# sabarim/STEm-Seg

Hardware: AMD Instinct MI355X
Metric: clips/sec (T=8, 480p) embed+cluster (higher is better)
Workload: dtype f16x3: fp32 emulated from 2 fp16 terms per operand (22-bit operand significands; fp32 has 24), power-of-two operand scaling, 3 fp16 MFMA products per fp32 product, fp32 accumulate; |activation| >= 2.6e5 -> non-finite, flagged on the device, clip re-run in bf16x6

## Files before the change

stem-seg_amd/csrc/conv_igemm.hip:

```cpp
#include "common.h"
#include <algorithm>
#include <cstdlib>
#include <type_traits>

#define STEMSEG_F16X3_ACT_SCALE 0.25f

#ifndef SS_F16_WPLANES
#define SS_F16_WPLANES 2
#endif
#ifndef SS_EXPERIMENTS
#if defined(SS_PROBE) || defined(SS_X6_WMODE_SMALLG) || defined(SS_X6_SPREAD) || defined(SS_X6_SPREAD_DIV)
#error "SS_PROBE / SS_X6_WMODE_SMALLG / SS_X6_SPREAD / SS_X6_SPREAD_DIV are experiment switches: add -DSS_EXPERIMENTS"
#endif
#define SS_X6_WMODE_SMALLG -1
#define SS_X6_SPREAD 1
#define SS_X6_SPREAD_DIV 1
#define SS_PROBE 0
#else
#ifndef SS_X6_WMODE_SMALLG
#define SS_X6_WMODE_SMALLG -1
#endif
#ifndef SS_X6_SPREAD
#define SS_X6_SPREAD 1
#endif
#ifndef SS_X6_SPREAD_DIV
#define SS_X6_SPREAD_DIV 1
#endif

#ifndef SS_PROBE
#define SS_PROBE 0
#endif

#endif

#if SS_PROBE == 5
#define SS_CHUNK_SYNC() do { } while (0)
#else
#define SS_CHUNK_SYNC() __syncthreads()
#endif

namespace stemseg {

typedef float f32x16 __attribute__((ext_vector_type(16)));

#ifndef STEMSEG_MIN_WG4
#define STEMSEG_MIN_WG4 4
#endif
constexpr int MIN_WG4 = STEMSEG_MIN_WG4;

struct ConvKParams {
    const float* in;
    int64_t in_cs, in_ts, in_ys, in_limit;
    int in_H;
    const float* wpk;
    const float* bias;
    float* out;
    int64_t out_cs, out_ts, out_ys;
    int Cin, Cout, T, H, W;
    int tiles_x, tiles_y;
    int vec4;
    int chunks_per_split;
    int64_t out_split_stride;
    int relu;
    const float* res;
    int64_t res_cs, res_ts, res_ys;
    int dec_H, dec_W;
    int vec_epi;
    int t_fastest;
    int flat_t;
    int T_all;
    int n_co;
    double* gn_part;
    int gn_cpg, gn_cap, gn_slot0;
    int* gn_used_host;
    int nb;
    int64_t in_bs, out_bs, gn_bs;
    unsigned int* out_p16;
};

template <int KT_, int KH_, int KW_, int CK_, int MI_, int NI_, int WM_, int WN_, int COLS_, bool PIPE_ = false, int BF_ = 0, bool DB_ = false,
          int PMAX_ = 0, bool GL_ = false, int BLK_ = 0>
struct ConvCfg {
    static constexpr bool PIPE = PIPE_, BF = BF_ != 0, X6 = BF_ >= 2, F16 = BF_ == 3, DB = DB_, FLAT = PMAX_ > 0, GL = GL_;
    static_assert(BF_ == 0 || BF_ == 2 || BF_ == 3, "precision: 0 fp32-input MFMA, 2 bf16x6, 3 f16x3");
    static constexpr int NPL = BF_ == 2 ? 3 : (BF_ == 3 ? SS_F16_WPLANES : 2);
    static constexpr int NPA = 3;
    static constexpr int NPX = BF_ == 2 ? 3 : 2;
    static constexpr int NPROD = BF_ == 2 ? 6 : 3;
    static constexpr int PMAX = PMAX_;
    static constexpr int KT = KT_, KH = KH_, KW = KW_, CK = CK_, MI = MI_, NI = NI_, WM = WM_, WN = WN_, COLS = COLS_;
    static constexpr int TAPS = KT * KH * KW;
    static constexpr int NTHREADS = 64 * WM * WN;
    static constexpr int MT = WM * MI * 32;
    static constexpr int NSEG = WN * NI;
    static constexpr bool BLK = BLK_ > 0;
    static constexpr int NLIVE = BLK ? BLK_ * COLS_ : NSEG;
    static constexpr int ROWS = BLK ? 4 * BLK_ : NSEG / COLS;
    static constexpr int TW = BLK ? 8 * COLS_ : COLS_ * 32;
    static constexpr int RH = ROWS + KH - 1;
    static constexpr int XL = (TW + KW - 1 + 3) / 4;
    static constexpr int XP = BLK ? ((4 * XL + 23) / 32) * 32 + 8 : 4 * XL;
    static constexpr int NT = NSEG * 32;
    static constexpr int FL = NT + 2 * PMAX + 8;
    static constexpr int IN_CH_STRIDE = FLAT ? KT * FL : KT * RH * XP;
    static constexpr int IN_PAIR_STRIDE = PMAX_ > 0 ? KT * (WN_ * NI_ * 32 + 2 * PMAX_ + 8) : KT * RH * XP;
    static constexpr int IN_PLANE_STRIDE = (CK / 2) * IN_PAIR_STRIDE;
    static constexpr int IN_FLOATS = X6 ? NPX * IN_PLANE_STRIDE : CK * IN_CH_STRIDE;
    static constexpr int TPG = TAPS >= 27 ? 4 : ((TAPS >= 9 && CK_ < 16) ? 2 : 1);
    static constexpr int CPH = 8 / TPG;
    static constexpr int NTG = (TAPS + TPG - 1) / TPG;
    static constexpr int NCG = BF ? CK / (2 * CPH) : 1;
    static constexpr int G = NTG * NCG;
    static constexpr int W_FLOATS = BF ? NPL * G * 2 * MT * 4 : CK * TAPS * MT;
    static constexpr int GA = (G + 1) / 2;
    static constexpr int WMODE = (BF_ >= 2 && G <= 2) ? (SS_X6_WMODE_SMALLG >= 0 ? SS_X6_WMODE_SMALLG : (BF_ == 3 ? 1 : ((WM * WN >= 8 || MI * NI < 8) ? 2 : 0))) : 0;
    static constexpr bool SP = WMODE == 1, LA = WMODE == 2;
    static constexpr int IN_ALL = IN_FLOATS;
    static constexpr int BUF_FLOATS = IN_ALL + W_FLOATS;
    static constexpr int LDS_FLOATS = BUF_FLOATS * (DB ? 2 : 1);
    static_assert(!BF || CK % (2 * CPH) == 0, "split-staged: a chunk holds whole k-groups");
    static_assert(BLK || NSEG % COLS == 0, "segments must fill whole rows");
    static_assert(!BLK || (BF_ >= 2 && PMAX_ == 0 && NI_ == 2 && NLIVE <= NSEG && NLIVE > NSEG - NI_ && XP % 32 == 8 && XP >= 4 * XL), "block tiles: split-staged, the last wave may lack its second block");
    static_assert(CK % 4 == 0 || (DB && GL_ && CK == 2 && !BF), "channel chunk is a multiple of the packed sub-chunk (4), or one channel pair (GL)");
    static_assert(LDS_FLOATS * 4 <= (X6 ? 160 : 80) * 1024, "two workgroups per CU (x6 eight-wave tiles: one)");
    static_assert(!X6 || (!DB && !GL && G >= 2 && CK % 2 == 0), "x6: 2-D / 3-D tiles, two weight phases");
    static_assert(!FLAT || (KH == 3 && KW == 3 && PMAX % 4 == 0), "flat tiles: 3x3 taps");
    static_assert(DB == GL_, "two LDS buffers are the direct-to-LDS form");
    static_assert(!GL || (DB && !BF), "direct-to-LDS staging is the double-buffered fp32 form");
    static constexpr int NWAVES = WM * WN;
    static constexpr int MIN_WG = X6 ? (MI * NI > 8 ? 1 : NWAVES >= 8 ? 2 : (LDS_FLOATS * 4 * 2 <= 160 * 1024 ? NWAVES / 2 : NWAVES / 4))
                                     : ((GL && LDS_FLOATS * 4 * 4 <= 140 * 1024 && MI * NI <= 4) ? MIN_WG4 : ((GL && LDS_FLOATS * 4 * 3 <= 160 * 1024) ? 3 : 2));
};

__device__ __forceinline__ void split_pair_f16(const float x0, const float x1, unsigned int& hw, unsigned int& lw) {
    const float qs = STEMSEG_F16X3_ACT_SCALE, ks = 2048.0f;
    unsigned int h, l;
    float r0, r1;
    asm("v_fma_mixlo_f16 %0, %1, %2, 0" : "=v"(h) : "v"(x0), "s"(qs));
    asm("v_fma_mixhi_f16 %0, %1, %2, 0" : "+v"(h) : "v"(x1), "s"(qs));
    asm("v_fma_mix_f32 %0, %1, %2, -%3 op_sel_hi:[0,0,1]" : "=v"(r0) : "v"(x0), "s"(qs), "v"(h));
    asm("v_fma_mix_f32 %0, %1, %2, -%3 op_sel:[0,0,1] op_sel_hi:[0,0,1]" : "=v"(r1) : "v"(x1), "s"(qs), "v"(h));
    asm("v_fma_mixlo_f16 %0, %1, %2, 0" : "=v"(l) : "v"(r0), "s"(ks));
    asm("v_fma_mixhi_f16 %0, %1, %2, 0" : "+v"(l) : "v"(r1), "s"(ks));
    hw = h;
    lw = l;
}

template <class C>
__global__ __launch_bounds__(C::NTHREADS, C::MIN_WG) void conv_igemm_kernel(const ConvKParams p) {
    __shared__ __attribute__((aligned(16))) float smem[C::LDS_FLOATS];
    float* const in_lds = smem;
    float* const w_lds = smem + C::IN_ALL;

    const int tid = threadIdx.x;
    const int lane = tid & 63;
    const int wave = __builtin_amdgcn_readfirstlane(tid >> 6);
    const int wm = wave / C::WN, wn = wave % C::WN;
    const int half = lane >> 5, l31 = lane & 31;

    int bx;
    {
        const int nwg = gridDim.x, xcd = blockIdx.x & 7, q = nwg >> 3, r = nwg & 7;
        bx = (xcd < r ? xcd * (q + 1) : r * (q + 1) + (xcd - r) * q) + (blockIdx.x >> 3);
    }
    const int co_tile = bx % p.n_co;
    bx /= p.n_co;
    int tx, ty, t;
    if (C::KT > 1 && p.t_fastest) {
        t = bx % p.T;
        bx /= p.T;
        tx = bx % p.tiles_x;
        ty = bx / p.tiles_x;
    } else {
        tx = bx % p.tiles_x;
        bx /= p.tiles_x;
        ty = bx % p.tiles_y;
        t = bx / p.tiles_y;
    }
    const int x0 = C::FLAT ? 0 : tx * C::TW, y0 = C::FLAT ? 0 : ty * C::ROWS;
    auto seg_row = [](const int sN, const int l) __attribute__((always_inline)) { return C::BLK ? (sN / C::COLS) * 4 + (l >> 3) : sN / C::COLS; };
    auto seg_col = [](const int sN, const int l) __attribute__((always_inline)) { return C::BLK ? (sN % C::COLS) * 8 + (l & 7) : (sN % C::COLS) * 32 + l; };
    const bool ni1_live = !C::BLK || (wn * C::NI + 1 < C::NLIVE);
    const int pitch = (int)p.in_ys;
    const int F0 = pitch + tx * C::NT;
    const int co0 = co_tile * C::MT;

    f32x16 acc[C::MI][C::NI];
#pragma unroll
    for (int mi = 0; mi < C::MI; ++mi)
#pragma unroll
        for (int ni = 0; ni < C::NI; ++ni)
#pragma unroll
            for (int r = 0; r < 16; ++r) acc[mi][ni][r] = 0.f;

    const float* a_ptr = w_lds + half * C::MT + wm * (C::MI * 32) + l31;
    const float* b_ptr[C::NI];
#pragma unroll
    for (int ni = 0; ni < C::NI; ++ni) {
        const int s = wn * C::NI + ni;
        b_ptr[ni] = C::FLAT ? in_lds + half * C::IN_CH_STRIDE + s * 32 + l31 + 3
                            : in_lds + half * C::IN_CH_STRIDE + seg_row(s, l31) * C::XP + seg_col(s, l31);
    }

    const unsigned int* b_ptr6[C::NI];
#pragma unroll
    for (int ni = 0; ni < C::NI; ++ni) {
        const int s = wn * C::NI + ni;
        b_ptr6[ni] = C::FLAT ? reinterpret_cast<const unsigned int*>(in_lds) + half * (C::CPH / 2) * C::IN_PAIR_STRIDE + s * 32 + l31 + 3
                             : reinterpret_cast<const unsigned int*>(in_lds) + half * (C::CPH / 2) * C::IN_PAIR_STRIDE + seg_row(min(s, C::NLIVE - 1), l31) * C::XP + seg_col(min(s, C::NLIVE - 1), l31);
    }
    const float* in_tile = p.in + (int64_t)blockIdx.y * p.in_bs + (int64_t)t * p.in_ts + x0;
    const int64_t tile_base = (int64_t)t * p.in_ts + x0;

    constexpr int XQ = C::XP / 4;
    constexpr int NQ = C::FLAT ? C::IN_FLOATS / 4 : C::CK * C::KT * C::RH * XQ;
    constexpr int MQ = C::MT / 4;
    constexpr int NWQ = C::BF ? C::NPL * C::G * 2 * C::MT : C::CK * C::TAPS * MQ;
    constexpr int IN_PT = (NQ + C::NTHREADS - 1) / C::NTHREADS, W_PT = (NWQ + C::NTHREADS - 1) / C::NTHREADS;
    auto fetch_in = [&](int c0, int q) -> float4 {
        if constexpr (C::FLAT) {
            constexpr int FQ = C::FL / 4;
            const int j4 = q % FQ, rr = q / FQ, dt = rr % C::KT, c = rr / C::KT;
            const int f = F0 - pitch - 4 + 4 * j4;
            const int64_t rel = (int64_t)(c0 + c) * p.in_cs + (int64_t)dt * p.in_ts + f;
            float4 v = make_float4(0.f, 0.f, 0.f, 0.f);
            if (c0 + c < p.Cin && f >= 0 && 4 * j4 < C::NT + 2 * pitch + 8 && tile_base + rel + 4 <= p.in_limit)
                v = *reinterpret_cast<const float4*>(in_tile + rel);
            return v;
        }
        const int xq = q % XQ;
        int rr = q / XQ;
        const int r = rr % C::RH;
        rr /= C::RH;
        const int dt = rr % C::KT;
        const int c = rr / C::KT;
        const int yy = min(y0 + r, p.in_H - 1);
        const int64_t rel = (int64_t)(c0 + c) * p.in_cs + (int64_t)dt * p.in_ts + (int64_t)yy * p.in_ys + xq * 4;
        float4 v = make_float4(0.f, 0.f, 0.f, 0.f);
        if (c0 + c < p.Cin && tile_base + rel + 4 <= p.in_limit) v = *reinterpret_cast<const float4*>(in_tile + rel);
        return v;
    };
    auto fetch_w = [&](int c0, int q) -> float4 {
        const int mq = q % MQ;
        if constexpr (C::CK == 2) {
            const int row2 = q / MQ, tap = row2 >> 1, e = row2 & 1;
            const float* wsrc2 = p.wpk + ((int64_t)(c0 / 4) * (C::TAPS * 4) + tap * 4 + ((c0 >> 1) & 1) * 2 + e) * p.Cout + co0;
            float4 v2 = make_float4(0.f, 0.f, 0.f, 0.f);
            if (c0 + e < p.Cin && co0 + mq * 4 < p.Cout) v2 = *reinterpret_cast<const float4*>(wsrc2 + mq * 4);
            return v2;
        }
        const int row = q / MQ;
        const int ch = c0 + (row / (C::TAPS * 4)) * 4 + (row & 3);
        const float* wsrc = p.wpk + (int64_t)(c0 / 4) * (C::TAPS * 4) * p.Cout + co0;
        float4 v = make_float4(0.f, 0.f, 0.f, 0.f);
        if (ch < p.Cin && co0 + mq * 4 < p.Cout) v = *reinterpret_cast<const float4*>(wsrc + (int64_t)row * p.Cout + mq * 4);
        return v;
    };
    auto addr_in = [&](int c0, int q) -> const float* {
        int64_t rel;
        if constexpr (C::FLAT) {
            constexpr int FQ = C::FL / 4;
            const int j4 = q % FQ, rr = q / FQ, dt = rr % C::KT, c = rr / C::KT;
            const int f = max(F0 - pitch - 4 + 4 * j4, 0);
            rel = (int64_t)(c0 + c) * p.in_cs + (int64_t)dt * p.in_ts + f;
        } else {
            const int xq = q % XQ;
            int rr = q / XQ;
            const int r = rr % C::RH;
            rr /= C::RH;
            const int dt = rr % C::KT;
            const int c = rr / C::KT;
            const int yy = min(y0 + r, p.in_H - 1);
            rel = (int64_t)(c0 + c) * p.in_cs + (int64_t)dt * p.in_ts + (int64_t)yy * p.in_ys + xq * 4;
        }
        const int64_t last = p.in_limit - 4 - tile_base;
        return in_tile + (rel < last ? rel : last);
    };
    auto addr_w = [&](int c0, int q) -> const float* {
        const int mq = q % MQ;
        if constexpr (C::CK == 2) {
            const int row2 = q / MQ, tap = row2 >> 1, e = row2 & 1;
            return p.wpk + ((int64_t)(c0 / 4) * (C::TAPS * 4) + tap * 4 + ((c0 >> 1) & 1) * 2 + e) * p.Cout + co0 + mq * 4;
        } else {
            const int row = q / MQ;
            return p.wpk + (int64_t)(c0 / 4) * (C::TAPS * 4) * p.Cout + co0 + (int64_t)row * p.Cout + mq * 4;
        }
    };
    auto glds_chunk = [&](int c0, const int off) {
        typedef const __attribute__((address_space(1))) void* gptr_t;
        typedef __attribute__((address_space(3))) void* lptr_t;
#pragma unroll
        for (int k = 0; k < IN_PT; ++k) {
            const int q = tid + k * C::NTHREADS;
            if (q < NQ) __builtin_amdgcn_global_load_lds((gptr_t)addr_in(c0, q), (lptr_t)(in_lds + off + (q - lane) * 4), 16, 0, 0);
        }
#pragma unroll
        for (int k = 0; k < W_PT; ++k) {
            const int q = tid + k * C::NTHREADS;
            if (q < NWQ) __builtin_amdgcn_global_load_lds((gptr_t)addr_w(c0, q), (lptr_t)(w_lds + off + (q - lane) * 4), 16, 0, 0);
        }
    };
    auto stage_direct = [&](int c0) {
        if (p.vec4) {
            for (int q = tid; q < NQ; q += C::NTHREADS) *reinterpret_cast<float4*>(in_lds + q * 4) = fetch_in(c0, q);
        } else if constexpr (!C::FLAT) {
            constexpr int NE = C::CK * C::KT * C::RH * C::XP;
            for (int q = tid; q < NE; q += C::NTHREADS) {
                const int xx = q % C::XP;
                int rr = q / C::XP;
                const int r = rr % C::RH;
                rr /= C::RH;
                const int dt = rr % C::KT;
                const int c = rr / C::KT;
                const int yy = min(y0 + r, p.in_H - 1);
                const int64_t rel = (int64_t)(c0 + c) * p.in_cs + (int64_t)dt * p.in_ts + (int64_t)yy * p.in_ys + xx;
                float v = 0.f;
                if (c0 + c < p.Cin && tile_base + rel < p.in_limit) v = in_tile[rel];
                in_lds[q] = v;
            }
        }
        for (int q = tid; q < NWQ; q += C::NTHREADS) *reinterpret_cast<float4*>(w_lds + q * 4) = fetch_w(c0, q);
    };

    auto split3 = [](const float x, unsigned int& h, unsigned int& m, unsigned int& l) {
        if constexpr (C::F16) {
            const float xs = x * STEMSEG_F16X3_ACT_SCALE;
            const _Float16 fh = (_Float16)xs;
            const _Float16 fl = (_Float16)((xs - (float)fh) * 2048.0f);
            h = *reinterpret_cast<const unsigned short*>(&fh);
            m = *reinterpret_cast<const unsigned short*>(&fl);
            l = 0;
        } else {
            const __bf16 bh = (__bf16)x;
            const float r1 = x - (float)bh;
            const __bf16 bm = (__bf16)r1;
            const __bf16 bl = (__bf16)(r1 - (float)bm);
            h = *reinterpret_cast<const unsigned short*>(&bh);
            m = *reinterpret_cast<const unsigned short*>(&bm);
            l = *reinterpret_cast<const unsigned short*>(&bl);
        }
    };
    constexpr int FQ6 = C::FL / 4;
    constexpr int XL6 = C::XL;
    constexpr int NQ6 = C::FLAT ? (C::CK / 2) * C::KT * FQ6 : (C::CK / 2) * C::KT * C::RH * XL6;
    auto in6_lds = [](const int q) __attribute__((always_inline)) { return C::BLK ? (q / XL6) * C::XP + (q % XL6) * 4 : q * 4; };
    constexpr int IN_PT6 = C::X6 ? (NQ6 + C::NTHREADS - 1) / C::NTHREADS : 1;
    constexpr int NWQ_A = C::NPL * C::GA * 2 * C::MT, NWQ6 = C::NPL * C::G * 2 * C::MT;
    auto in6_rel = [&](int q, int& c) -> int64_t {
        if constexpr (C::FLAT) {
            const int j4 = q % FQ6, rr = q / FQ6, dt = rr % C::KT;
            c = 2 * (rr / C::KT);
            const int f = F0 - pitch - 4 + 4 * j4;
            if (f < 0 || 4 * j4 >= C::NT + 2 * pitch + 8) return -1;
            return (int64_t)c * p.in_cs + (int64_t)dt * p.in_ts + f;
        }
        const int xq = q % XL6;
        int rr = q / XL6;
        const int r = rr % C::RH;
        rr /= C::RH;
        const int dt = rr % C::KT;
        c = 2 * (rr / C::KT);
        const int yy = min(y0 + r, p.in_H - 1);
        return (int64_t)c * p.in_cs + (int64_t)dt * p.in_ts + (int64_t)yy * p.in_ys + xq * 4;
    };
    auto fetch_in6 = [&](int c0, int q, float4& v0, float4& v1) {
        int c;
        const int64_t rel0 = in6_rel(q, c);
        const int64_t rel = rel0 + (int64_t)c0 * p.in_cs;
        v0 = v1 = make_float4(0.f, 0.f, 0.f, 0.f);
        if (rel0 < 0) return;
        if (c0 + c < p.Cin && tile_base + rel + 4 <= p.in_limit) v0 = *reinterpret_cast<const float4*>(in_tile + rel);
        if (c0 + c + 1 < p.Cin && tile_base + rel + p.in_cs + 4 <= p.in_limit) v1 = *reinterpret_cast<const float4*>(in_tile + rel + p.in_cs);
    };
    unsigned int in6_voff[IN_PT6];
    int in6_clim[IN_PT6];
    const int64_t in6_room = (p.in_limit - 4 - tile_base) * 4;
    if constexpr (C::X6) {
#pragma unroll
        for (int k = 0; k < IN_PT6; ++k) {
            const int q = tid + k * C::NTHREADS;
            int c = 0;
            const int64_t rel0 = q < NQ6 ? in6_rel(q, c) : 0;
            const int64_t rel = rel0 < 0 ? 0 : rel0;
            in6_voff[k] = (unsigned int)(rel * 4);
            const int64_t slack = in6_room - rel * 4;
            const int64_t by_room = slack < 0 ? 0 : slack / (p.in_cs * 4) + 1;
            in6_clim[k] = (q < NQ6 && rel0 >= 0) ? (int)min((int64_t)(p.Cin - c), by_room) : 0;
        }
    }
    typedef float f32x4 __attribute__((ext_vector_type(4)));
    auto fetch_in6_fast = [&](int c0, int k, f32x4& v0, f32x4& v1) __attribute__((always_inline)) {
#if SS_PROBE == 1
        return;
#endif
        const char* base = reinterpret_cast<const char*>(in_tile) + (int64_t)c0 * p.in_cs * 4;
        const unsigned int cs4 = (unsigned int)(p.in_cs * 4);
        v0 = *reinterpret_cast<const f32x4*>(base + (c0 < in6_clim[k] ? in6_voff[k] : 0u));
        v1 = *reinterpret_cast<const f32x4*>(base + (c0 + 1 < in6_clim[k] ? in6_voff[k] + cs4 : 0u));
    };
    auto store_in6 = [&](int q, const float4& v0, const float4& v1) {
        unsigned int h0, m0, l0, h1, m1, l1;
        uint4 ph, pm, pl;
        if constexpr (C::F16) {
            split_pair_f16(v0.x, v1.x, ph.x, pm.x); split_pair_f16(v0.y, v1.y, ph.y, pm.y);
            split_pair_f16(v0.z, v1.z, ph.z, pm.z); split_pair_f16(v0.w, v1.w, ph.w, pm.w);
            unsigned int* d16 = reinterpret_cast<unsigned int*>(in_lds) + in6_lds(q);
            *reinterpret_cast<uint4*>(d16) = ph;
            *reinterpret_cast<uint4*>(d16 + C::IN_PLANE_STRIDE) = pm;
            return;
        }
        split3(v0.x, h0, m0, l0); split3(v1.x, h1, m1, l1); ph.x = h0 | (h1 << 16); pm.x = m0 | (m1 << 16); pl.x = l0 | (l1 << 16);
        split3(v0.y, h0, m0, l0); split3(v1.y, h1, m1, l1); ph.y = h0 | (h1 << 16); pm.y = m0 | (m1 << 16); pl.y = l0 | (l1 << 16);
        split3(v0.z, h0, m0, l0); split3(v1.z, h1, m1, l1); ph.z = h0 | (h1 << 16); pm.z = m0 | (m1 << 16); pl.z = l0 | (l1 << 16);
        split3(v0.w, h0, m0, l0); split3(v1.w, h1, m1, l1); ph.w = h0 | (h1 << 16); pm.w = m0 | (m1 << 16); pl.w = l0 | (l1 << 16);
        unsigned int* d = reinterpret_cast<unsigned int*>(in_lds) + in6_lds(q);
        *reinterpret_cast<uint4*>(d) = ph;
        *reinterpret_cast<uint4*>(d + C::IN_PLANE_STRIDE) = pm;
        if constexpr (C::NPX == 3) *reinterpret_cast<uint4*>(d + 2 * C::IN_PLANE_STRIDE) = pl;
    };
    auto store_in6_masked = [&](int c0, int k, const f32x4& r0, const f32x4& r1) __attribute__((always_inline)) {
        const bool ok0 = c0 < in6_clim[k], ok1 = c0 + 1 < in6_clim[k];
        float4 v0, v1;
        v0.x = ok0 ? r0.x : 0.f; v0.y = ok0 ? r0.y : 0.f; v0.z = ok0 ? r0.z : 0.f; v0.w = ok0 ? r0.w : 0.f;
        v1.x = ok1 ? r1.x : 0.f; v1.y = ok1 ? r1.y : 0.f; v1.z = ok1 ? r1.z : 0.f; v1.w = ok1 ? r1.w : 0.f;
        store_in6(tid + k * C::NTHREADS, v0, v1);
    };
    auto stage_in6_direct = [&](int c0) {
        if (p.vec4) {
            for (int q = tid; q < NQ6; q += C::NTHREADS) {
                float4 v0, v1;
                fetch_in6(c0, q, v0, v1);
                store_in6(q, v0, v1);
            }
        } else if constexpr (!C::FLAT) {
            constexpr int NE6 = (C::CK / 2) * C::KT * C::RH * C::XP;
            for (int q = tid; q < NE6; q += C::NTHREADS) {
                const int xx = q % C::XP;
                int rr = q / C::XP;
                const int r = rr % C::RH;
                rr /= C::RH;
                const int dt = rr % C::KT;
                const int c = 2 * (rr / C::KT);
                const int yy = min(y0 + r, p.in_H - 1);
                const int64_t rel = (int64_t)(c0 + c) * p.in_cs + (int64_t)dt * p.in_ts + (int64_t)yy * p.in_ys + xx;
                float a0 = 0.f, a1 = 0.f;
                if (c0 + c < p.Cin && tile_base + rel < p.in_limit) a0 = in_tile[rel];
                if (c0 + c + 1 < p.Cin && tile_base + rel + p.in_cs < p.in_limit) a1 = in_tile[rel + p.in_cs];
                unsigned int h0, m0, l0, h1, m1, l1;
                split3(a0, h0, m0, l0);
                split3(a1, h1, m1, l1);
                unsigned int* d = reinterpret_cast<unsigned int*>(in_lds) + q;
                d[0] = h0 | (h1 << 16);
                d[C::IN_PLANE_STRIDE] = m0 | (m1 << 16);
                if constexpr (C::NPX == 3) d[2 * C::IN_PLANE_STRIDE] = l0 | (l1 << 16);
            }
        }
    };
    constexpr int W_PT6 = C::X6 ? ((C::SP ? NWQ6 : NWQ_A) + C::NTHREADS - 1) / C::NTHREADS : 1;
    static_assert(C::NTHREADS % C::MT == 0 && NWQ_A % C::MT == 0, "weight pieces: a thread keeps its column");
    const unsigned int w6_voff = C::X6 ? ((unsigned int)(tid / C::MT) * (unsigned int)p.Cout + (unsigned int)min(tid % C::MT, p.Cout - 1 - co0)) * 16u : 0u;
    auto w6_src = [&](int c0, int q_uniform) __attribute__((always_inline)) -> const char* {
        const char* base = reinterpret_cast<const char*>(p.wpk) +
                           (((int64_t)(c0 / C::CK) * (C::NPL * C::G * 2) + q_uniform / C::MT) * p.Cout + co0) * 16;
        return base + w6_voff;
    };
    auto compute6 = [&](auto g0c, auto g1c, auto&& side, auto live_c) __attribute__((always_inline)) {
        constexpr int g0 = decltype(g0c)::value, g1 = decltype(g1c)::value;
        constexpr bool LIVE1 = decltype(live_c)::value;
        constexpr int NPL = C::NPL, NPX = C::NPX, NPA = C::NPA;
        typedef typename std::conditional<C::F16, _Float16, __bf16>::type h16;
        typedef h16 h16x8 __attribute__((ext_vector_type(8)));
        const char* a_base = reinterpret_cast<const char*>(w_lds) + (half * C::MT + wm * (C::MI * 32) + l31) * 16;
        const unsigned int* bdy6[C::NI][3];
        if constexpr (C::FLAT) {
#pragma unroll
            for (int ni = 0; ni < C::NI; ++ni) { bdy6[ni][0] = b_ptr6[ni]; bdy6[ni][1] = b_ptr6[ni] + pitch; bdy6[ni][2] = b_ptr6[ni] + 2 * pitch; }
        }
        auto ld_b = [&](const int grp, h16x8 (&b)[NPX][C::NI]) __attribute__((always_inline)) {
#if SS_PROBE == 4
            if (grp >= 0) { _Pragma("unroll") for (int pl = 0; pl < NPX; ++pl) _Pragma("unroll") for (int ni = 0; ni < C::NI; ++ni) asm volatile("" : "+v"(b[pl][ni])); return; }
#endif
            const int cg = grp / C::NTG, tg = grp % C::NTG;
#pragma unroll
            for (int ni = 0; ni < (LIVE1 ? C::NI : 1); ++ni)
#pragma unroll
                for (int pl = 0; pl < NPX; ++pl) {
                    uint4 w4;
                    unsigned int* wv = reinterpret_cast<unsigned int*>(&w4);
#pragma unroll
                    for (int wd = 0; wd < 4; ++wd) {
                        const int j0 = 2 * wd, tapi = j0 / C::CPH, chl = j0 % C::CPH;
                        int tap = tg * C::TPG + tapi;
                        tap = tap < C::TAPS ? tap : C::TAPS - 1;
                        const int dt = tap / (C::KH * C::KW), dy = (tap / C::KW) % C::KH, dx = tap % C::KW;
                        if constexpr (C::FLAT) {
                            const int off = pl * C::IN_PLANE_STRIDE + (cg * C::CPH + chl / 2) * C::IN_PAIR_STRIDE + dt * C::FL + dx;
                            wv[wd] = bdy6[ni][dy][off];
                        } else {
                            const int off = pl * C::IN_PLANE_STRIDE + (cg * C::CPH + chl / 2) * C::IN_PAIR_STRIDE + (dt * C::RH + dy) * C::XP + dx;
                            wv[wd] = b_ptr6[ni][off];
                        }
                    }
                    b[pl][ni] = __builtin_bit_cast(h16x8, w4);
                }
        };
        auto ld_a = [&](const int grp, const int mi, h16x8 (&a)[NPA]) __attribute__((always_inline)) {
#if SS_PROBE == 4
            if (grp >= 0) { _Pragma("unroll") for (int pl = 0; pl < NPL; ++pl) asm volatile("" : "+v"(a[pl])); return; }
#endif
#pragma unroll
            for (int pl = 0; pl < NPL; ++pl)
                a[pl] = *reinterpret_cast<const h16x8*>(a_base + (((grp * NPL + pl) * 2) * C::MT + mi * 32) * 16);
        };
        auto mm = [&](const int mi, h16x8 (&a)[NPA], const h16x8 (&b)[NPX][C::NI]) __attribute__((always_inline)) {
#if SS_PROBE == 3
            _Pragma("unroll") for (int pl = 0; pl < NPL; ++pl) asm volatile("" ::"v"(a[pl]));
            _Pragma("unroll") for (int pl = 0; pl < NPX; ++pl) _Pragma("unroll") for (int ni = 0; ni < C::NI; ++ni) asm volatile("" ::"v"(b[pl][ni]));
            return;
#endif
            if constexpr (C::F16) {
                if constexpr (NPL == 2) a[2] = a[0] * (h16)(1.0f / 2048.0f);
#define SS_X6_TERM(PA, PB)                                                                                                     \
    _Pragma("unroll") for (int ni = 0; ni < (LIVE1 ? C::NI : 1); ++ni)                                                         \
        acc[mi][ni] = __builtin_amdgcn_mfma_f32_32x32x16_f16(a[PA], b[PB][ni], acc[mi][ni], 0, 0, 0);
                SS_X6_TERM(1, 0) SS_X6_TERM(2, 1) SS_X6_TERM(0, 0)
#undef SS_X6_TERM
            } else {
#define SS_X6_TERM(PA, PB)                                                                                                     \
    _Pragma("unroll") for (int ni = 0; ni < (LIVE1 ? C::NI : 1); ++ni)                                                         \
        acc[mi][ni] = __builtin_amdgcn_mfma_f32_32x32x16_bf16(a[PA], b[PB][ni], acc[mi][ni], 0, 0, 0);
                SS_X6_TERM(2, 0) SS_X6_TERM(0, 2) SS_X6_TERM(1, 1) SS_X6_TERM(1, 0) SS_X6_TERM(0, 1) SS_X6_TERM(0, 0)
#undef SS_X6_TERM
            }
        };
        constexpr int NSTEP = (g1 - g0) * C::MI;
        h16x8 bfr[NPX][C::NI], a0[NPA], a1[NPA];
        side(-1);
        ld_b(g0, bfr);
        ld_a(g0, 0, a0);
#pragma unroll
        for (int st = 0; st < NSTEP; st += 2) {
            const int grp = g0 + st / C::MI, mi = st % C::MI;
            if (st + 1 < NSTEP) ld_a(g0 + (st + 1) / C::MI, (st + 1) % C::MI, a1);
            side(st);
            __builtin_amdgcn_sched_barrier(0);
            mm(mi, a0, bfr);
            __builtin_amdgcn_sched_barrier(0);
            if (st + 1 < NSTEP) {
                if ((st + 1) % C::MI == 0) ld_b(g0 + (st + 1) / C::MI, bfr);
                if (st + 2 < NSTEP) ld_a(g0 + (st + 2) / C::MI, (st + 2) % C::MI, a0);
                side(st + 1);
                __builtin_amdgcn_sched_barrier(0);
                mm((st + 1) % C::MI, a1, bfr);
                __builtin_amdgcn_sched_barrier(0);
                if (st + 2 < NSTEP && (st + 2) % C::MI == 0) ld_b(g0 + (st + 2) / C::MI, bfr);
            }
            (void)grp;
        }
    };
    auto compute = [&](const int buf_off = 0) {
        constexpr int NSUB = C::CK >= 4 ? C::CK / 4 : 1, NCP = C::CK >= 4 ? 2 : 1, WROWS = C::CK >= 4 ? 4 : 2;
        const float* bdy[C::NI][3];
        if constexpr (C::FLAT) {
#pragma unroll
            for (int ni = 0; ni < C::NI; ++ni) {
                bdy[ni][0] = b_ptr[ni]; bdy[ni][1] = b_ptr[ni] + pitch; bdy[ni][2] = b_ptr[ni] + 2 * pitch;
            }
        }
        constexpr int NSTEPS = NSUB * C::TAPS * NCP;
        auto ld = [&](const int i, float (&a)[C::MI], float (&b)[C::NI]) {
            const int cp = i % NCP, tap = (i / NCP) % C::TAPS, sub = i / (NCP * C::TAPS);
            const int dt = tap / (C::KH * C::KW), dy = (tap / C::KW) % C::KH, dx = tap % C::KW;
            const int wrow = (sub * C::TAPS + tap) * WROWS + cp * 2;
            const int boff = C::FLAT ? (sub * 4 + cp * 2) * C::IN_CH_STRIDE + dt * C::FL + dx
                                     : (sub * 4 + cp * 2) * C::IN_CH_STRIDE + (dt * C::RH + dy) * C::XP + dx;
#pragma unroll
            for (int mi = 0; mi < C::MI; ++mi) a[mi] = a_ptr[buf_off + wrow * C::MT + mi * 32];
#pragma unroll
            for (int ni = 0; ni < C::NI; ++ni) {
                if constexpr (C::FLAT) b[ni] = bdy[ni][dy][buf_off + boff];
                else b[ni] = b_ptr[ni][buf_off + boff];
            }
        };
        auto mm = [&](const float (&a)[C::MI], const float (&b)[C::NI]) {
#pragma unroll
            for (int mi = 0; mi < C::MI; ++mi)
#pragma unroll
                for (int ni = 0; ni < C::NI; ++ni)
                    acc[mi][ni] = __builtin_amdgcn_mfma_f32_32x32x2f32(a[mi], b[ni], acc[mi][ni], 0, 0, 0);
        };
        float a0[C::MI], b0[C::NI], a1[C::MI], b1[C::NI];
        ld(0, a0, b0);
#pragma unroll
        for (int i = 0; i < NSTEPS; i += 2) {
            if (i + 1 < NSTEPS) ld(i + 1, a1, b1);
            __builtin_amdgcn_sched_barrier(0);
            mm(a0, b0);
            __builtin_amdgcn_sched_barrier(0);
            if (i + 1 < NSTEPS) {
                if (i + 2 < NSTEPS) ld(i + 2, a0, b0);
                __builtin_amdgcn_sched_barrier(0);
                mm(a1, b1);
                __builtin_amdgcn_sched_barrier(0);
            }
        }
    };

    const int c_begin = blockIdx.z * p.chunks_per_split * C::CK;
    const int c_end = min(p.Cin, c_begin + p.chunks_per_split * C::CK);
    if constexpr (C::X6) {
        typedef std::integral_constant<int, 0> Q0;
        typedef std::integral_constant<int, NWQ_A> QA;
        typedef std::integral_constant<int, NWQ6> QE;
        f32x4 rin[2 * IN_PT6];
        f32x4 rw6[W_PT6];
        f32x4 rw6b[W_PT6];
        auto fetch_w6_k = [&](int c0, auto q0c, auto q1c, f32x4 (&r)[W_PT6], const int k) __attribute__((always_inline)) {
            constexpr int q0 = decltype(q0c)::value, q1 = decltype(q1c)::value;
#if SS_PROBE == 1
            return;
#endif
            if ((k + 1) * C::NTHREADS <= q1 - q0 || q0 + tid + k * C::NTHREADS < q1) r[k] = *reinterpret_cast<const f32x4*>(w6_src(c0, q0 + k * C::NTHREADS));
        };
        auto store_w6 = [&](auto q0c, auto q1c, const f32x4 (&r)[W_PT6]) __attribute__((always_inline)) {
            constexpr int q0 = decltype(q0c)::value, q1 = decltype(q1c)::value;
#if SS_PROBE == 2
            _Pragma("unroll") for (int k = 0; k < W_PT6; ++k) asm volatile("" ::"v"(r[k]));
            return;
#endif
    #pragma unroll
            for (int k = 0; k < W_PT6; ++k) { const int q = q0 + tid + k * C::NTHREADS; if ((k + 1) * C::NTHREADS <= q1 - q0 || (k * C::NTHREADS < q1 - q0 && q < q1)) *reinterpret_cast<f32x4*>(w_lds + q * 4) = r[k]; }
        };
        auto store_in6_all = [&](int c0) __attribute__((always_inline)) {
#if SS_PROBE == 2
            _Pragma("unroll") for (int k = 0; k < 2 * IN_PT6; ++k) asm volatile("" ::"v"(rin[k]));
            return;
#endif
            if (p.vec4) {
#pragma unroll
                for (int k = 0; k < IN_PT6; ++k) {
                    const int q = tid + k * C::NTHREADS;
                    if ((k + 1) * C::NTHREADS <= NQ6 || q < NQ6) store_in6_masked(c0, k, rin[2 * k], rin[2 * k + 1]);
                }
            } else stage_in6_direct(c0);
        };
        auto side_items = [&](const int st, auto nspread_c, auto n_in_c, auto n_w_c, auto&& f_in, auto&& f_w) __attribute__((always_inline)) {
            constexpr int nspread = decltype(nspread_c)::value, n_in = decltype(n_in_c)::value, n_w = decltype(n_w_c)::value, n = n_in + n_w;
            if (st >= nspread || st < 0) return;
#pragma unroll
            for (int i = 0; i < n; ++i)
                if (i >= st * n / nspread && i < (st + 1) * n / nspread) { if (i < n_in) f_in(i); else f_w(i - n_in); }
        };
        constexpr int NSA = C::GA * C::MI, NSB = (C::G - C::GA) * C::MI, NSALL = C::G * C::MI;
        constexpr int NPA = (NWQ_A + C::NTHREADS - 1) / C::NTHREADS, NPB = (NWQ6 - NWQ_A + C::NTHREADS - 1) / C::NTHREADS;
        constexpr int NPALL = (NWQ6 + C::NTHREADS - 1) / C::NTHREADS;
        constexpr bool SPRD = SS_X6_SPREAD && (C::F16 || SS_X6_SPREAD > 1);
        typedef std::integral_constant<int, C::GA> GAc;
        typedef std::integral_constant<int, C::G> Gc;
        typedef std::integral_constant<int, 0> I0;
        typedef std::integral_constant<int, IN_PT6> INc;
        if (c_begin < c_end) {
            for (int q = tid; q < NWQ6; q += C::NTHREADS) *reinterpret_cast<float4*>(w_lds + q * 4) = *reinterpret_cast<const float4*>(w6_src(c_begin, q - tid));
            stage_in6_direct(c_begin);
        }
        __syncthreads();
        typedef std::true_type Yes;
        typedef std::false_type No;
        auto f_in_at = [&](const int cn) { return [&, cn](const int k) __attribute__((always_inline)) { if (p.vec4) fetch_in6_fast(cn, k, rin[2 * k], rin[2 * k + 1]); }; };
        if constexpr (C::SP) {
            auto chunk = [&](const int c0, auto more_c) __attribute__((always_inline)) {
                constexpr bool more = decltype(more_c)::value;
                const int cn = c0 + C::CK;
                compute6(Q0{}, Gc{}, [&](const int st) __attribute__((always_inline)) {
                    if constexpr (more) {
                        side_items(SPRD ? st : -1 - st, std::integral_constant<int, SPRD ? (NSALL + SS_X6_SPREAD_DIV - 1) / SS_X6_SPREAD_DIV : 1>{}, INc{}, std::integral_constant<int, NPALL>{}, f_in_at(cn),
                                   [&](const int k) __attribute__((always_inline)) { fetch_w6_k(cn, Q0{}, QE{}, rw6, k); });
                    }
                }, Yes{});
                SS_CHUNK_SYNC();
                if constexpr (more) {
                    store_w6(Q0{}, QE{}, rw6);
                    store_in6_all(cn);
                    SS_CHUNK_SYNC();
                }
            };
            int c0 = c_begin;
            for (; c0 + C::CK < c_end; c0 += C::CK) chunk(c0, Yes{});
            if (c0 < c_end) chunk(c0, No{});
        } else if constexpr (C::LA) {
            if (c_begin + C::CK < c_end) {
#pragma unroll
                for (int k = 0; k < NPA; ++k) fetch_w6_k(c_begin + C::CK, Q0{}, QA{}, rw6, k);
            }
            auto chunk = [&](const int c0, auto more_c, auto more2_c) __attribute__((always_inline)) {
                constexpr bool more = decltype(more_c)::value, more2 = decltype(more2_c)::value;
                const int cn = c0 + C::CK, cnn = c0 + 2 * C::CK;
                compute6(Q0{}, GAc{}, [&](const int st) __attribute__((always_inline)) {
                    if constexpr (more) side_items(SPRD ? st : -1 - st, std::integral_constant<int, SPRD ? NSA : 1>{}, INc{}, std::integral_constant<int, NPB>{}, f_in_at(cn),
                                         [&](const int k) __attribute__((always_inline)) { fetch_w6_k(cn, QA{}, QE{}, rw6b, k); });
                }, Yes{});
                SS_CHUNK_SYNC();
                if constexpr (more) store_w6(Q0{}, QA{}, rw6);
                compute6(GAc{}, Gc{}, [&](const int st) __attribute__((always_inline)) {
                    if constexpr (more2) side_items(SPRD ? st : -1 - st, std::integral_constant<int, SPRD ? (NSB + SS_X6_SPREAD_DIV - 1) / SS_X6_SPREAD_DIV : 1>{}, I0{}, std::integral_constant<int, NPA>{}, [](const int) {},
                                          [&](const int k) __attribute__((always_inline)) { fetch_w6_k(cnn, Q0{}, QA{}, rw6, k); });
                }, Yes{});
                SS_CHUNK_SYNC();
                if constexpr (more) {
                    store_w6(QA{}, QE{}, rw6b);
                    store_in6_all(cn);
                    SS_CHUNK_SYNC();
                }
            };
            int c0 = c_begin;
            for (; c0 + 2 * C::CK < c_end; c0 += C::CK) chunk(c0, Yes{}, Yes{});
            if (c0 + C::CK < c_end) { chunk(c0, Yes{}, No{}); c0 += C::CK; }
            if (c0 < c_end) chunk(c0, No{}, No{});
        } else {
            auto chunk = [&](const int c0, auto more_c, auto live_c) __attribute__((always_inline)) {
                constexpr bool more = decltype(more_c)::value;
                const int cn = c0 + C::CK;
                compute6(Q0{}, GAc{}, [&](const int st) __attribute__((always_inline)) {
                    if constexpr (more) side_items(SPRD ? st : -1 - st, std::integral_constant<int, SPRD ? (NSA + SS_X6_SPREAD_DIV - 1) / SS_X6_SPREAD_DIV : 1>{}, INc{}, std::integral_constant<int, NPA>{}, f_in_at(cn),
                                         [&](const int k) __attribute__((always_inline)) { fetch_w6_k(cn, Q0{}, QA{}, rw6, k); });
                }, live_c);
                SS_CHUNK_SYNC();
                if constexpr (more) store_w6(Q0{}, QA{}, rw6);
                compute6(GAc{}, Gc{}, [&](const int st) __attribute__((always_inline)) {
                    if constexpr (more) {
                        side_items(SPRD ? st : -1 - st, std::integral_constant<int, SPRD ? (NSB + SS_X6_SPREAD_DIV - 1) / SS_X6_SPREAD_DIV : 1>{}, I0{}, std::integral_constant<int, NPB>{}, [](const int) {},
                                   [&](const int k) __attribute__((always_inline)) { fetch_w6_k(cn, QA{}, QE{}, rw6, k); });
                    }
                }, live_c);
                SS_CHUNK_SYNC();
                if constexpr (more) {
                    store_w6(QA{}, QE{}, rw6);
                    store_in6_all(cn);
                    SS_CHUNK_SYNC();
                }
            };
            auto run = [&](auto live_c) __attribute__((always_inline)) {
                int c0 = c_begin;
                for (; c0 + C::CK < c_end; c0 += C::CK) chunk(c0, Yes{}, live_c);
                if (c0 < c_end) chunk(c0, No{}, live_c);
            };
            if constexpr (C::BLK && C::NLIVE < C::NSEG) {
                if (ni1_live) run(Yes{});
                else run(No{});
            } else run(Yes{});
        }
        if constexpr (C::F16) {
            const float* invp = reinterpret_cast<const float*>(reinterpret_cast<const char*>(p.wpk) +
                                                               (int64_t)((p.Cin + C::CK - 1) / C::CK) * (C::NPL * C::G * 2) * p.Cout * 16);
            const int co_w = co0 + wm * (C::MI * 32) + 4 * half;
#pragma unroll
            for (int mi = 0; mi < C::MI; ++mi)
#pragma unroll
                for (int j = 0; j < 4; ++j) {
                    const int co4 = co_w + mi * 32 + 8 * j;
                    const float4 sc = co4 < p.Cout ? *reinterpret_cast<const float4*>(invp + co4) : make_float4(1.f, 1.f, 1.f, 1.f);
#pragma unroll
                    for (int ni = 0; ni < C::NI; ++ni) {
                        acc[mi][ni][4 * j + 0] *= sc.x; acc[mi][ni][4 * j + 1] *= sc.y;
                        acc[mi][ni][4 * j + 2] *= sc.z; acc[mi][ni][4 * j + 3] *= sc.w;
                    }
                }
        }
    } else if constexpr (C::DB && C::GL) {
        if (c_begin < c_end) glds_chunk(c_begin, 0);
        __syncthreads();
        int cur = 0;
        for (int c0 = c_begin; c0 < c_end; c0 += C::CK) {
            if (c0 + C::CK < c_end) glds_chunk(c0 + C::CK, C::BUF_FLOATS - cur);
            __builtin_amdgcn_sched_barrier(0);
            compute(cur);
            cur = C::BUF_FLOATS - cur;
            __syncthreads();
        }
    } else if (C::PIPE && p.vec4) {
        float4 rin[IN_PT], rw[W_PT];
        auto fetch_regs = [&](int c0) {
#pragma unroll
            for (int k = 0; k < IN_PT; ++k) { const int q = tid + k * C::NTHREADS; if (q < NQ) rin[k] = fetch_in(c0, q); }
#pragma unroll
            for (int k = 0; k < W_PT; ++k) { const int q = tid + k * C::NTHREADS; if (q < NWQ) rw[k] = fetch_w(c0, q); }
        };
        auto regs_to_lds = [&]() {
#pragma unroll
            for (int k = 0; k < IN_PT; ++k) { const int q = tid + k * C::NTHREADS; if (q < NQ) *reinterpret_cast<float4*>(in_lds + q * 4) = rin[k]; }
#pragma unroll
            for (int k = 0; k < W_PT; ++k) { const int q = tid + k * C::NTHREADS; if (q < NWQ) *reinterpret_cast<float4*>(w_lds + q * 4) = rw[k]; }
        };
        if (c_begin < c_end) {
            fetch_regs(c_begin);
            regs_to_lds();
        }
        __syncthreads();
        for (int c0 = c_begin; c0 < c_end; c0 += C::CK) {
            const bool more = c0 + C::CK < c_end;
            if (more) fetch_regs(c0 + C::CK);
            __builtin_amdgcn_sched_barrier(0);
            compute();
            __syncthreads();
            if (more) {
                regs_to_lds();
                __syncthreads();
            }
        }
    } else {
        for (int c0 = c_begin; c0 < c_end; c0 += C::CK) {
            __syncthreads();
            stage_direct(c0);
            __syncthreads();
            compute();
        }
    }

    const int co_base = co0 + wm * (C::MI * 32);
    if (p.gn_part) {
        __syncthreads();
        constexpr int GPW8 = C::MI * 4;
        double* red = reinterpret_cast<double*>(smem + C::NWAVES * 32 * 36);
        static_assert(C::NWAVES * 32 * 36 + 2 * C::WM * C::WN * GPW8 * 2 * 2 <= C::LDS_FLOATS, "GN partial sums must fit the staging LDS");
        const bool g4 = p.gn_cpg == 4;
        bool ok[C::NI];
#pragma unroll
        for (int ni = 0; ni < C::NI; ++ni) {
            const int sN = wn * C::NI + ni;
            int y = y0 + seg_row(sN, l31), x = x0 + seg_col(sN, l31);
            if constexpr (C::FLAT) {
                const int f = F0 + sN * 32 + l31, y1 = f / pitch, x1 = f - y1 * pitch;
                y = y1 - 1;
                x = (x1 >= 1) ? x1 - 1 : p.W;
            }
            ok[ni] = y < p.H && x < p.W && sN < C::NLIVE;
        }
#pragma unroll
        for (int mi = 0; mi < C::MI; ++mi) {
#pragma unroll
            for (int j = 0; j < 4; ++j) {
                float fs = 0.f, fss = 0.f;
#pragma unroll
                for (int rr = 0; rr < 4; ++rr) {
                    const int co = co_base + mi * 32 + rr + 8 * j + 4 * half;
                    const float bv = (p.bias && co < p.Cout) ? p.bias[co] : 0.f;
#pragma unroll
                    for (int ni = 0; ni < C::NI; ++ni)
                        if (ok[ni]) {
                            const float v = acc[mi][ni][4 * j + rr] + bv;
                            fs += v;
                            fss += v * v;
                        }
                }
                double ds = (double)fs, dss = (double)fss;
#pragma unroll
                for (int o = 16; o > 0; o >>= 1) { ds += __shfl_xor(ds, o, 64); dss += __shfl_xor(dss, o, 64); }
                if (!g4) { ds += __shfl_xor(ds, 32, 64); dss += __shfl_xor(dss, 32, 64); }
                if (l31 == 0 && (g4 || half == 0)) {
                    const int gl = g4 ? (mi * 4 + j) * 2 + half : mi * 4 + j;
                    const int gpw = g4 ? 2 * GPW8 : GPW8;
                    double* d = red + ((size_t)(wm * gpw + gl) * C::WN + wn) * 2;
                    d[0] = ds; d[1] = dss;
                }
            }
        }
        __syncthreads();
        {
            const int gpw = g4 ? 2 * GPW8 : GPW8, ngw = C::WM * gpw;
            if (tid < ngw) {
                double a = 0.0, b = 0.0;
#pragma unroll
                for (int k = 0; k < C::WN; ++k) { a += red[((size_t)tid * C::WN + k) * 2]; b += red[((size_t)tid * C::WN + k) * 2 + 1]; }
                const int gg = co0 / p.gn_cpg + tid;
                if (gg * p.gn_cpg < p.Cout) {
                    const int slot = p.gn_slot0 + (t * p.tiles_y + ty) * p.tiles_x + tx;
                    double* o = p.gn_part + (int64_t)blockIdx.y * p.gn_bs + ((size_t)gg * p.gn_cap + slot) * 2;
                    o[0] = a; o[1] = b;
                }
            }
        }
        __syncthreads();
    }
    if (p.vec_epi && !C::FLAT) {
        __syncthreads();
        constexpr int TP = 36;
        float* tl = smem + wave * (32 * TP);
        static_assert(C::NWAVES * 32 * 36 <= C::LDS_FLOATS, "epilogue transpose buffer must fit the staging LDS");
#pragma unroll
        for (int ni = 0; ni < C::NI; ++ni) {
            const int s = wn * C::NI + ni;
            if (C::BLK && s >= C::NLIVE) continue;
            const int y = y0 + seg_row(s, (lane & 7) * 4);
            const int xs = x0 + seg_col(s, (lane & 7) * 4) - (lane & 7) * 4;
            constexpr int MG = (C::MI >= 2 && C::MIN_WG < 3) ? 2 : 1;
#pragma unroll
            for (int m0 = 0; m0 < C::MI; m0 += MG) {
                float4 rres[MG][4];
                float rbias[MG][4];
#pragma unroll
                for (int mg = 0; mg < MG; ++mg)
#pragma unroll
                    for (int j = 0; j < 4; ++j) {
                        const int row = (lane >> 3) + 8 * j, c4 = (lane & 7) * 4;
                        const int co = co_base + (m0 + mg) * 32 + row;
                        const int x = xs + c4;
                        rres[mg][j] = make_float4(0.f, 0.f, 0.f, 0.f);
                        rbias[mg][j] = 0.f;
                        if (y < p.H && x < p.W && co < p.Cout) {
                            if (p.res) rres[mg][j] = *reinterpret_cast<const float4*>(p.res + (int64_t)co * p.res_cs + (int64_t)t * p.res_ts + (int64_t)y * p.res_ys + x);
                            if (p.bias) rbias[mg][j] = p.bias[co];
                        }
                    }
#pragma unroll
                for (int mg = 0; mg < MG; ++mg) {
                    const int mi = m0 + mg;
#pragma unroll
                    for (int r = 0; r < 16; ++r) tl[((r & 3) + 8 * (r >> 2) + 4 * half) * TP + l31] = acc[mi][ni][r];
                    __builtin_amdgcn_s_waitcnt(0xc07f);
#pragma unroll
                    for (int j = 0; j < 4; ++j) {
                        const int row = (lane >> 3) + 8 * j, c4 = (lane & 7) * 4;
                        const int co = co_base + mi * 32 + row;
                        const int x = xs + c4;
                        if (y < p.H && x < p.W && co < p.Cout) {
                            float4 v = *reinterpret_cast<const float4*>(tl + row * TP + c4);
                            const float bv = rbias[mg][j];
                            v.x += bv; v.y += bv; v.z += bv; v.w += bv;
                            const int64_t off = (int64_t)t * p.out_ts + (int64_t)y * p.out_ys + x;
                            const float4 rv = rres[mg][j];
                            v.x += rv.x; v.y += rv.y; v.z += rv.z; v.w += rv.w;
                            if (p.relu) { v.x = relu_keep_nan(v.x); v.y = relu_keep_nan(v.y); v.z = relu_keep_nan(v.z); v.w = relu_keep_nan(v.w); }
                            *reinterpret_cast<float4*>(p.out + (int64_t)blockIdx.y * p.out_bs + (int64_t)blockIdx.z * p.out_split_stride + (int64_t)co * p.out_cs + off) = v;
                        }
                    }
                    __builtin_amdgcn_s_waitcnt(0xc07f);
                }
            }
        }
        return;
    }
#pragma unroll
    for (int ni = 0; ni < C::NI; ++ni) {
        const int s = wn * C::NI + ni;
        if (C::BLK && s >= C::NLIVE) continue;
        int y = y0 + seg_row(s, l31);
        int x = x0 + seg_col(s, l31);
        int te = t;
        if constexpr (C::FLAT) {
            int f = F0 + s * 32 + l31;
            if (p.flat_t) {
                te = f / (int)p.in_ts;
                f -= te * (int)p.in_ts;
            }
            const int y1 = f / pitch, x1 = f - y1 * pitch;
            y = (y1 >= 1 && te < p.T_all) ? y1 - 1 : p.H;
            x = (x1 >= 1) ? x1 - 1 : p.W;
        }
        if (y < p.H && x < p.W) {
            int64_t off, roff = 0;
            if (p.dec_W > 0) {
                const int hw = p.dec_H * p.dec_W;
                const int t2 = x / hw, r2 = x - t2 * hw, y2 = r2 / p.dec_W, x2 = r2 - y2 * p.dec_W;
                off = (int64_t)t2 * p.out_ts + (int64_t)y2 * p.out_ys + x2;
                roff = (int64_t)t2 * p.res_ts + (int64_t)y2 * p.res_ys + x2;
            } else {
                off = (int64_t)te * p.out_ts + (int64_t)y * p.out_ys + x;
                roff = (int64_t)te * p.res_ts + (int64_t)y * p.res_ys + x;
            }
            if constexpr (C::F16) {
                if (p.out_p16) {
                    const int64_t plane_words = (int64_t)(p.Cout / 8) * p.out_cs * 4;
#pragma unroll
// ... 753 lines not shown
```

Before: 123.5.

## Stream f16x3 conv weights into LDS with direct global-to-LDS DMA per phase

For f16 x6 tiles in the default weight mode, weight slabs are now fetched with global_load_lds straight into LDS instead of through registers. The schedule changes to match: while the first weight phase is being consumed, the second phase of the current chunk is DMA'd in, and during the second phase the first phase of the next chunk is loaded. This removes the register staging and the store_w6 pass, which should lower VGPR pressure and cut the sync-heavy store step. The risk is LDS write hazards on phase buffers shared across the two syncs, plus a new requirement that MT be a multiple of 64.

Result: no change. 123.1 (median of 2 runs) (-0.3%).

```diff
diff --git a/stem-seg_amd/csrc/conv_igemm.hip b/stem-seg_amd/csrc/conv_igemm.hip
--- a/stem-seg_amd/csrc/conv_igemm.hip
+++ b/stem-seg_amd/csrc/conv_igemm.hip
@@ -7,6 +7,9 @@
 
 #ifndef SS_F16_WPLANES
 #define SS_F16_WPLANES 2
+#endif
+#ifndef SS_F16_WDMA
+#define SS_F16_WDMA 1
 #endif
 #ifndef SS_EXPERIMENTS
 #if defined(SS_PROBE) || defined(SS_X6_WMODE_SMALLG) || defined(SS_X6_SPREAD) || defined(SS_X6_SPREAD_DIV)
@@ -115,6 +118,7 @@
     static constexpr int GA = (G + 1) / 2;
     static constexpr int WMODE = (BF_ >= 2 && G <= 2) ? (SS_X6_WMODE_SMALLG >= 0 ? SS_X6_WMODE_SMALLG : (BF_ == 3 ? 1 : ((WM * WN >= 8 || MI * NI < 8) ? 2 : 0))) : 0;
     static constexpr bool SP = WMODE == 1, LA = WMODE == 2;
+    static constexpr bool WDMA = F16 && SS_F16_WDMA && WMODE == 0;
     static constexpr int IN_ALL = IN_FLOATS;
     static constexpr int BUF_FLOATS = IN_ALL + W_FLOATS;
     static constexpr int LDS_FLOATS = BUF_FLOATS * (DB ? 2 : 1);
@@ -127,6 +131,7 @@
     static_assert(!FLAT || (KH == 3 && KW == 3 && PMAX % 4 == 0), "flat tiles: 3x3 taps");
     static_assert(DB == GL_, "two LDS buffers are the direct-to-LDS form");
     static_assert(!GL || (DB && !BF), "direct-to-LDS staging is the double-buffered fp32 form");
+    static_assert(!WDMA || MT % 64 == 0, "weight DMA: a wave's 64 pieces lie in one slab row of one phase");
     static constexpr int NWAVES = WM * WN;
     static constexpr int MIN_WG = X6 ? (MI * NI > 8 ? 1 : NWAVES >= 8 ? 2 : (LDS_FLOATS * 4 * 2 <= 160 * 1024 ? NWAVES / 2 : NWAVES / 4))
                                      : ((GL && LDS_FLOATS * 4 * 4 <= 140 * 1024 && MI * NI <= 4) ? MIN_WG4 : ((GL && LDS_FLOATS * 4 * 3 <= 160 * 1024) ? 3 : 2));
@@ -659,15 +664,55 @@
         typedef std::integral_constant<int, C::G> Gc;
         typedef std::integral_constant<int, 0> I0;
         typedef std::integral_constant<int, IN_PT6> INc;
+        constexpr int NWQ_PRO = C::WDMA ? NWQ_A : NWQ6;
         if (c_begin < c_end) {
-            for (int q = tid; q < NWQ6; q += C::NTHREADS) *reinterpret_cast<float4*>(w_lds + q * 4) = *reinterpret_cast<const float4*>(w6_src(c_begin, q - tid));
+            for (int q = tid; q < NWQ_PRO; q += C::NTHREADS) *reinterpret_cast<float4*>(w_lds + q * 4) = *reinterpret_cast<const float4*>(w6_src(c_begin, q - tid));
             stage_in6_direct(c_begin);
         }
         __syncthreads();
+        auto dma_w6_k = [&](int c0, auto q0c, auto q1c, const int k) __attribute__((always_inline)) {
+            constexpr int q0 = decltype(q0c)::value, q1 = decltype(q1c)::value;
+            typedef const __attribute__((address_space(1))) void* gptr_t;
+            typedef __attribute__((address_space(3))) void* lptr_t;
+            const int qw = q0 + k * C::NTHREADS + wave * 64;
+            if ((k + 1) * C::NTHREADS <= q1 - q0 || qw < q1)
+                __builtin_amdgcn_global_load_lds((gptr_t)w6_src(c0, q0 + k * C::NTHREADS), (lptr_t)(w_lds + qw * 4), 16, 0, 0);
+        };
         typedef std::true_type Yes;
         typedef std::false_type No;
         auto f_in_at = [&](const int cn) { return [&, cn](const int k) __attribute__((always_inline)) { if (p.vec4) fetch_in6_fast(cn, k, rin[2 * k], rin[2 * k + 1]); }; };
-        if constexpr (C::SP) {
+        if constexpr (C::WDMA) {
+            auto chunk = [&](const int c0, auto more_c, auto live_c) __attribute__((always_inline)) {
+                constexpr bool more = decltype(more_c)::value;
+                const int cn = c0 + C::CK;
+                compute6(Q0{}, GAc{}, [&](const int st) __attribute__((always_inline)) {
+                    side_items(SPRD ? st : -1 - st, std::integral_constant<int, SPRD ? (NSA + SS_X6_SPREAD_DIV - 1) / SS_X6_SPREAD_DIV : 1>{}, std::integral_constant<int, NPB>{},
+                               std::integral_constant<int, more ? IN_PT6 : 0>{},
+                               [&](const int k) __attribute__((always_inline)) { dma_w6_k(c0, QA{}, QE{}, k); }, f_in_at(cn));
+                }, live_c);
+                SS_CHUNK_SYNC();
+                compute6(GAc{}, Gc{}, [&](const int st) __attribute__((always_inline)) {
+                    if constexpr (more) {
+                        side_items(SPRD ? st : -1 - st, std::integral_constant<int, SPRD ? (NSB + SS_X6_SPREAD_DIV - 1) / SS_X6_SPREAD_DIV : 1>{}, std::integral_constant<int, NPA>{}, I0{},
+                                   [&](const int k) __attribute__((always_inline)) { dma_w6_k(cn, Q0{}, QA{}, k); }, [](const int) {});
+                    }
+                }, live_c);
+                SS_CHUNK_SYNC();
+                if constexpr (more) {
+                    store_in6_all(cn);
+                    SS_CHUNK_SYNC();
+                }
+            };
+            auto run = [&](auto live_c) __attribute__((always_inline)) {
+                int c0 = c_begin;
+                for (; c0 + C::CK < c_end; c0 += C::CK) chunk(c0, Yes{}, live_c);
+                if (c0 < c_end) chunk(c0, No{}, live_c);
+            };
+            if constexpr (C::BLK && C::NLIVE < C::NSEG) {
+                if (ni1_live) run(Yes{});
+                else run(No{});
+            } else run(Yes{});
+        } else if constexpr (C::SP) {
             auto chunk = [&](const int c0, auto more_c) __attribute__((always_inline)) {
                 constexpr bool more = decltype(more_c)::value;
                 const int cn = c0 + C::CK;
```
